# endernewton/tf-faster-rcnn

Measured on AMD Instinct MI355X. Metric: images/sec (600×1000) ResNet-101 Faster R-CNN at 1/2/4/8 MI355X, higher is better.
Workload: dtype f32 (operands, accumulators, results; GEMMs with Cin, Cout % 128 == 0 form each f32 product from two-piece fp16 operands with an exact power-of-two scale per 128-k block on the fp16 matrix pipe -- 3 MFMAs / product, dropped terms <= 3 * 2^-22, measured error vs float64 below the f32-MFMA kernel's; o

## Files before the change

### scratch/h2_conv3.py

```python
import os, sys
ROOT = os.path.dirname(os.path.dirname(os.path.abspath(__file__)))
sys.path[:0] = [os.path.join(ROOT, "tf-faster-rcnn_amd")]
args = [a for a in sys.argv[1:]]
lib_path, single = None, 0
if "--lib" in args:
    i = args.index("--lib"); lib_path = args[i + 1]; del args[i:i + 2]
if "--single" in args:
    i = args.index("--single"); single = int(args[i + 1]); del args[i:i + 2]
import frcnn_hip
if lib_path:
    frcnn_hip.LIB_PATH = os.path.abspath(lib_path)
import numpy as np, torch
from frcnn_hip import ops
dev = torch.device("cuda:0")
shapes = {
    "b4c3x8":  (1, 117600, 2048, 512, True, True, True, 0),
    "b4c3x8m": (8, 14700, 2048, 512, True, False, False, 49),
    "b4c3x8pm": (8, 14700, 2048, 512, "planes", False, False, 49),
    "b3c3x8":  (1, 19152, 1024, 256, True, True, True, 0),
    "b2c3x8":  (1, 75000, 512, 128, True, True, True, 0),
    "b4c3x8p": (1, 117600, 2048, 512, "planes", False, True, 0),
    "b3c3x8p": (1, 19152, 1024, 256, "planes", False, True, 0),
    "b3scx8":  (1, 19152, 1024, 512, False, True, True, 0),
    "w7x8":    (121, 2400, 512, 512, False, True, False, 0),
    "w3x8":    (36, 1280, 256, 256, False, True, False, 0),
    "wrpnx8":  (36, 1280, 512, 1024, False, True, False, 0),
    "b4c1x8":  (1, 117600, 512, 2048, False, False, True, 0),
    "b3c1x8":  (1, 19152, 256, 1024, False, True, False, 0),
    "cal_k128": (1, 117600, 128, 128, "planes", False, True, 0),
    "b4c3x1":  (1, 14700, 2048, 512, True, True, True, 0),
    "b3c3x1":  (1, 2394, 1024, 256, True, True, True, 0),
}
cfgs = [int(c) for c in (args[0] if args else "9,21,12").split(",")]
only = args[1].split(",") if len(args) > 1 else ["b4c3x8", "b4c3x8m", "b3c3x8", "b2c3x8", "w7x8", "w3x8", "b4c1x8", "b3c1x8"]
if not single:
    print("%-8s %-4s %9s %9s %8s %8s  %s" % ("shape", "cfg", "med_us", "min_us", "TFLOP/s", "GB/s", "bits vs cfg %d" % cfgs[0]))
for name in only:
    G, M, N, K, has_res, f32o, planes, mean_rows = shapes[name]
    torch.manual_seed(1)
    x = torch.randn(G * M, K, device=dev).clamp(min=0) * torch.exp(torch.rand(G * M, K, device=dev) * 4 - 2)
    shared_w = mean_rows > 0
    w = torch.randn(1 if shared_w else G, N, K, device=dev) * 0.05
    b = torch.randn(N, device=dev) if (G == 1 or shared_w) else None
    res = torch.randn(G * M, N, device=dev) if has_res else None
    if has_res == "planes":
        res = ops.h2_split(res.clamp(min=0))
    xp, wp = ops.h2_split(x), ops.h2_pack_w(w)
    del x
    outs, outp = {}, {}
    share = G * M * N * 4 > (1 << 29)
    for c in cfgs:
        if mean_rows:
            outs[c] = torch.empty(G * M // mean_rows, N, device=dev)
        else:
            outs[c] = (outs[cfgs[0]] if (share and c != cfgs[0]) else torch.empty(G * M, N, device=dev)) if f32o else None
            outp[c] = (outp[cfgs[0]] if (share and c != cfgs[0]) else ops.H2.empty(G * M, N, dev)) if planes else None

    def run(c):
        if mean_rows:
            return ops.gemm_h2_mean(xp, wp, G, M, N, K, b, res, 1, mean_rows, out=outs[c], cfg=c)
        return ops.gemm_h2(xp, wp, G, M, N, K, b, res, 1, out=outs[c], out_planes=outp.get(c), want_f32=f32o, cfg=c)

    if single:
        for _ in range(single):
            run(cfgs[0])
        torch.cuda.synchronize()
        break
    def digest(c):
        parts = []
        if outs.get(c) is not None:
            parts.append(outs[c].view(torch.int32).to(torch.int64).sum())
            parts.append((outs[c].view(torch.int32).to(torch.int64) * torch.arange(1, outs[c].numel() + 1, device=dev).view(outs[c].shape) % 1000003).sum())
        if outp.get(c) is not None:
            pv = outp[c].planes.view(torch.int16).to(torch.int64)
            parts.append(pv.sum()); parts.append((pv * (torch.arange(pv.numel(), device=dev) % 8191 + 1)).sum())
            parts.append(outp[c].inv.view(torch.int32).to(torch.int64).sum())
        return tuple(int(p) for p in parts)
    digs = {}
    for c in cfgs:
        if outs.get(c) is not None: outs[c].fill_(float("nan"))
        if outp.get(c) is not None: outp[c].planes.zero_(); outp[c].inv.zero_()
        try:
            run(c); torch.cuda.synchronize()
            digs[c] = digest(c)
        except Exception as e:
            digs[c] = "unsupported (%s)" % (str(e)[:60],)
    live = [c for c in cfgs if not isinstance(digs[c], str)]
    times = {c: [] for c in live}
    for r in range(6):
        for c in live:
            e0, e1 = torch.cuda.Event(enable_timing=True), torch.cuda.Event(enable_timing=True)
            e0.record()
            for _ in range(6): run(c)
            e1.record(); torch.cuda.synchronize()
            if r: times[c].append(e0.elapsed_time(e1) * 1000 / 6)
    nbytes = 4.0 * G * M * K + 4.0 * (w.numel()) + G * M * N * 4.0 * ((1 if has_res else 0) + (1 if f32o else 0) + (1 if planes else 0))
    for c in cfgs:
        if c not in live:
            print("%-8s %-4d %s" % (name, c, digs[c]), flush=True)
            continue
        med = float(np.median(times[c]))
        print("%-8s %-4d %9.1f %9.1f %8.1f %8.0f  %s" % (name, c, med, min(times[c]), 2.0 * G * M * N * K / med / 1e6, nbytes / med / 1e3,
                                                       "identical" if digs[c] == digs[cfgs[0]] else "DIFFERENT"), flush=True)
    del outs, outp, xp, res
    torch.cuda.empty_cache()
```

### tf-faster-rcnn_amd/csrc/gemm_h2.hip

```cpp
#include "h2_common.h"
#include <mutex>
#include <type_traits>

typedef float f32x16 __attribute__((ext_vector_type(16)));
typedef _Float16 h8 __attribute__((ext_vector_type(8)));

#define LDS_AS __attribute__((address_space(3)))

struct GemmH2Params {
  const unsigned short* x; const float* x_inv; const unsigned short* w; const float* w_inv;
  const float* bias; const float* res; const unsigned short* resp; const float* resp_inv; float* y; unsigned short* yp; float* y_inv;
  int M, N, K, batch, act, nsteps, mtiles, ntiles;
  long long Mtot;
  int wshare;
  const float* mask;
  float* mean_part; int mean_rows;
};

__device__ __forceinline__ void h2_glds16(unsigned voff, const void* sbase, unsigned lds_base) {
  unsigned keep;
  asm volatile(
      "s_mov_b32 %0, m0\n\t"
      "s_mov_b32 m0, %3\n\t"
      "s_nop 0\n\t"
// ... 318 lines not shown
  };

  int c_tile = tile0, c_step = 0, cur = 0, nxt = 0;
  int c_bm0 = 0, c_bn0 = 0, c_g = 0;
  auto set_ctile = [&](int tl) {
    int g, mt, nt;
    tile_coords(tl, g, mt, nt);
    c_bm0 = mt * BM; c_bn0 = nt * BN; c_g = g;
  };
  const float act_lo = p.act == FRCNN_ACT_NONE ? -__builtin_inff() : 0.f;
  const float act_hi = p.act == FRCNN_ACT_RELU6 ? 6.f : __builtin_inff();

  auto rsrc_f = [&](const void* base, long long elems_left, int esize) {
    const long long bytes = elems_left * esize;
    return __builtin_amdgcn_make_buffer_rsrc((void*)base, 0, (int)max(0ll, min(bytes, 0x7fffffffll)), 0x00020000);
  };

  struct TileRef { int bm0, bn0, g, cpar; };
  auto ent_rsrc = [&](const void* base, int g, int esize) {
    const char* b = (const char*)base + (size_t)g * p.M * p.N * esize;
    return __builtin_amdgcn_make_buffer_rsrc((void*)b, 0, p.M * p.N * esize, 0x00020000);
  };
  const int lo4 = (frow * p.N + 4 * khalf) * 4;
  auto lo2_of = [&]() { int v = lo4; asm volatile("" : "+v"(v)); return v >> 1; };
  auto lo2w_of = [&]() { int v = lo4; asm volatile("" : "+v"(v)); return (v >> 1) + 8 * (int)(threadIdx.x >> 5 & 1); };
  auto sub_off = [&](const auto& T, int i, int j) {
    return __builtin_amdgcn_readfirstlane((T.bm0 + wm0 + i * 32) * p.N + T.bn0 + wn0 + j * 32);
  };

  auto load_res_raw = [&](int i) {
    typedef unsigned u32x4 __attribute__((ext_vector_type(4)));
    const TileRef C{c_bm0, c_bn0, c_g, c_cpar};
    const bool planes = !p.res && p.resp;
    const auto none = __builtin_amdgcn_make_buffer_rsrc((void*)nullptr, 0, 0, 0x00020000);
    const auto r_even = p.res ? ent_rsrc(p.res, c_g, 4) : planes ? ent_rsrc(p.resp, c_g, 2) : none;
    const auto r_odd = p.res ? r_even : planes ? ent_rsrc(p.resp + (size_t)p.Mtot * p.N, c_g, 2) : none;
    const int step_q = planes ? 0 : 32, step_p = planes ? 32 : 0;
    int base = lo4;
    asm volatile("" : "+v"(base));
    if (planes) base = (base >> 1) + 8 * (int)(threadIdx.x >> 5 & 1);
#pragma unroll
    for (int j = 0; j < TN; ++j) {
      const int vo = base + sub_off(C, i, j) * (planes ? 2 : 4);
#pragma unroll
      for (int q = 0; q < 4; ++q) {
        const u32x4 ld = __builtin_amdgcn_raw_buffer_load_b128((q & 1) ? r_odd : r_even, vo, q * step_q + (q >> 1) * step_p, 0);
        tot[i][j][4 * q + 0] = __uint_as_float(ld[0]); tot[i][j][4 * q + 1] = __uint_as_float(ld[1]);
        tot[i][j][4 * q + 2] = __uint_as_float(ld[2]); tot[i][j][4 * q + 3] = __uint_as_float(ld[3]);
      }
      pend += 4;
    }
  };
  auto init_tot = [&]() {
    if constexpr (DE) return;
    if constexpr (LTB) {
      if (p.res || p.resp) {
#pragma unroll
        for (int i = 0; i < TM; ++i) load_res_raw(i);
      } else {
#pragma unroll
        for (int i = 0; i < TM; ++i)
#pragma unroll
          for (int j = 0; j < TN; ++j)
#pragma unroll
            for (int r = 0; r < 16; ++r) tot[i][j][r] = 0.f;
      }
      return;
    }
    const size_t row_base = (size_t)c_g * p.M;
    typedef unsigned u32x4 __attribute__((ext_vector_type(4)));
    if (p.res) {
#pragma unroll
      for (int i = 0; i < TM; ++i)
#pragma unroll
        for (int j = 0; j < TN; ++j) {
          const int m0 = c_bm0 + wm0 + i * 32, nc = c_bn0 + wn0 + j * 32;
          const auto rr = rsrc_f(p.res + (long long)(row_base + m0) * p.N + nc, (long long)(p.M - m0) * p.N - nc, 4);
#pragma unroll
          for (int q = 0; q < 4; ++q) {
            const u32x4 ld = __builtin_amdgcn_raw_buffer_load_b128(rr, (frow * p.N + 4 * khalf) * 4 + 32 * q, 0, 0);
            tot[i][j][4 * q + 0] = __uint_as_float(ld[0]); tot[i][j][4 * q + 1] = __uint_as_float(ld[1]);
            tot[i][j][4 * q + 2] = __uint_as_float(ld[2]); tot[i][j][4 * q + 3] = __uint_as_float(ld[3]);
          }
        }
      pend += TM * TN * 4;
    } else if (p.resp) {
      float ri[TM];
#pragma unroll
      for (int i = 0; i < TM; ++i)
        ri[i] = p.resp_inv[(size_t)(c_bn0 / H2_KB) * p.Mtot + row_base + min(c_bm0 + wm0 + i * 32 + frow, p.M - 1)];
      h4 hv[TM][TN][4], lv[TM][TN][4];
#pragma unroll
      for (int i = 0; i < TM; ++i)
#pragma unroll
        for (int j = 0; j < TN; ++j) {
          const int m0 = c_bm0 + wm0 + i * 32, nc = c_bn0 + wn0 + j * 32;
          const long long sbase = (long long)(row_base + m0) * p.N + nc, left_e = (long long)(p.M - m0) * p.N - nc;
          const auto rh = rsrc_f(p.resp + sbase, left_e, 2), rl = rsrc_f(p.resp + (size_t)p.Mtot * p.N + sbase, left_e, 2);
#pragma unroll
          for (int q = 0; q < 4; ++q) {
            const int lo2 = (frow * p.N + 4 * khalf) * 2 + 16 * q;
            hv[i][j][q] = __builtin_bit_cast(h4, __builtin_amdgcn_raw_buffer_load_b64(rh, lo2, 0, 0));
            lv[i][j][q] = __builtin_bit_cast(h4, __builtin_amdgcn_raw_buffer_load_b64(rl, lo2, 0, 0));
          }
        }
#pragma unroll
      for (int i = 0; i < TM; ++i)
#pragma unroll
        for (int j = 0; j < TN; ++j)
#pragma unroll
          for (int q = 0; q < 4; ++q)
#pragma unroll
            for (int e = 0; e < 4; ++e) tot[i][j][4 * q + e] = ((float)hv[i][j][q][e] + (float)lv[i][j][q][e]) * ri[i];
    } else {
#pragma unroll
      for (int i = 0; i < TM; ++i)
#pragma unroll
        for (int j = 0; j < TN; ++j)
#pragma unroll
          for (int r = 0; r < 16; ++r) tot[i][j][r] = 0.f;
    }
    float4 wi[TN][4], bv[TN][4];
#pragma unroll
    for (int j = 0; j < TN; ++j)
#pragma unroll
      for (int q = 0; q < 4; ++q)
        wi[j][q] = *(const float4*)(p.w_inv + (size_t)(p.wshare ? 0 : c_g) * p.N + c_bn0 + wn0 + j * 32 + 4 * khalf + 8 * q);
    if (p.bias) {
#pragma unroll
      for (int j = 0; j < TN; ++j)
#pragma unroll
        for (int q = 0; q < 4; ++q) bv[j][q] = *(const float4*)(p.bias + c_bn0 + wn0 + j * 32 + 4 * khalf + 8 * q);
    } else {
#pragma unroll
      for (int j = 0; j < TN; ++j)
#pragma unroll
        for (int q = 0; q < 4; ++q) bv[j][q] = make_float4(0.f, 0.f, 0.f, 0.f);
    }
#pragma unroll
    for (int j = 0; j < TN; ++j)
#pragma unroll
      for (int q = 0; q < 4; ++q) {
        const float s0 = __uint_as_float(0x7f000000u - __float_as_uint(wi[j][q].x)), s1 = __uint_as_float(0x7f000000u - __float_as_uint(wi[j][q].y));
        const float s2 = __uint_as_float(0x7f000000u - __float_as_uint(wi[j][q].z)), s3 = __uint_as_float(0x7f000000u - __float_as_uint(wi[j][q].w));
#pragma unroll
        for (int i = 0; i < TM; ++i) {
          tot[i][j][4 * q + 0] = (tot[i][j][4 * q + 0] + bv[j][q].x) * s0;
          tot[i][j][4 * q + 1] = (tot[i][j][4 * q + 1] + bv[j][q].y) * s1;
          tot[i][j][4 * q + 2] = (tot[i][j][4 * q + 2] + bv[j][q].z) * s2;
          tot[i][j][4 * q + 3] = (tot[i][j][4 * q + 3] + bv[j][q].w) * s3;
        }
      }
  };

  auto ep_scale_act = [&](const TileRef& T) {
#pragma unroll
    for (int j = 0; j < TN; ++j) {
      const int n0 = T.bn0 + wn0 + j * 32 + 4 * khalf;
#pragma unroll
      for (int q = 0; q < 4; ++q) {
        const float4 wi = LTB ? *(const float4*)(smem + CB_OFF + T.cpar * (2 * BN * 4) + (wn0 + j * 32 + 4 * khalf + 8 * q) * 4)
                             : *(const float4*)(p.w_inv + (size_t)(p.wshare ? 0 : T.g) * p.N + n0 + 8 * q);
#pragma unroll
        for (int i = 0; i < TM; ++i) {
          tot[i][j][4 * q + 0] = act_clamp(tot[i][j][4 * q + 0] * wi.x, act_lo, act_hi);
          tot[i][j][4 * q + 1] = act_clamp(tot[i][j][4 * q + 1] * wi.y, act_lo, act_hi);
          tot[i][j][4 * q + 2] = act_clamp(tot[i][j][4 * q + 2] * wi.z, act_lo, act_hi);
          tot[i][j][4 * q + 3] = act_clamp(tot[i][j][4 * q + 3] * wi.w, act_lo, act_hi);
        }
      }
    }
  };
  auto ep_mask = [&](const TileRef& T) {
    if (MASKED && p.mask) {
      const auto rk = ent_rsrc(p.mask, T.g, 4);
#pragma unroll
      for (int i = 0; i < TM; ++i)
#pragma unroll
        for (int j = 0; j < TN; ++j) {
          const int vo = lo4 + sub_off(T, i, j) * 4;
          typedef unsigned u32x4 __attribute__((ext_vector_type(4)));
          u32x4 k[4];
#pragma unroll
          for (int q = 0; q < 4; ++q) k[q] = __builtin_amdgcn_raw_buffer_load_b128(rk, vo + 32 * q, 0, 0);
#pragma unroll
          for (int q = 0; q < 4; ++q)
#pragma unroll
            for (int e = 0; e < 4; ++e) tot[i][j][4 * q + e] = __uint_as_float(k[q][e]) > 0.f ? tot[i][j][4 * q + e] : 0.f;
        }
      pend += TM * TN * 4;
    }
  };
  auto ep_mean = [&](const TileRef& T, int i) {
    const int mb = T.bm0 + wm0 + i * 32;
    if (mb >= p.M) return;
    const int nblk = (p.M + 31) >> 5;
    const int m = mb + frow, g0 = mb / p.mean_rows, gid = m / p.mean_rows;
    const bool in_a = m < p.M && gid == g0, in_b = m < p.M && gid == g0 + 1;
    const bool two = mb - g0 * p.mean_rows + 31 >= p.mean_rows;
    float* dst = p.mean_part + ((size_t)T.g * nblk + (mb >> 5)) * 2 * p.N;
#pragma unroll
    for (int j = 0; j < TN; ++j) {
      const int n0 = T.bn0 + wn0 + j * 32 + 4 * khalf;
#pragma unroll
      for (int q = 0; q < 4; ++q) {
        float a[4];
#pragma unroll
        for (int e = 0; e < 4; ++e) a[e] = h2_sum32(in_a ? tot[i][j][4 * q + e] : 0.f);
        if (frow == 0) *(float4*)(dst + n0 + 8 * q) = make_float4(a[0], a[1], a[2], a[3]);
        ++pend;
        if (two) {
          float b[4];
#pragma unroll
          for (int e = 0; e < 4; ++e) b[e] = h2_sum32(in_b ? tot[i][j][4 * q + e] : 0.f);
          if (frow == 0) *(float4*)(dst + p.N + n0 + 8 * q) = make_float4(b[0], b[1], b[2], b[3]);
          ++pend;
        }
      }
    }
  };
  auto ep_store_f32 = [&](const TileRef& T, int i) {
    if (!p.y) return;
    const auto ry = ent_rsrc(p.y, T.g, 4);
#pragma unroll
    for (int j = 0; j < TN; ++j) {
      const int lo = lo4 + sub_off(T, i, j) * 4;
#pragma unroll
      for (int q = 0; q < 4; ++q) {
        typedef unsigned u32x4 __attribute__((ext_vector_type(4)));
        u32x4 o;
        o[0] = __float_as_uint(tot[i][j][4 * q + 0]); o[1] = __float_as_uint(tot[i][j][4 * q + 1]);
        o[2] = __float_as_uint(tot[i][j][4 * q + 2]); o[3] = __float_as_uint(tot[i][j][4 * q + 3]);
        __builtin_amdgcn_raw_buffer_store_b128(o, ry, lo + 32 * q, 0, 0);
      }
      pend += 4;
      if constexpr (DE) __builtin_amdgcn_sched_barrier(0);
    }
  };
  auto ep_rowmax_write = [&](float (&mx)[TM]) {
    float* red = (float*)(smem + RED_OFF);
#pragma unroll
    for (int i = 0; i < TM; ++i) {
      float m = 0.f;
#pragma unroll
      for (int j = 0; j < TN; ++j)
#pragma unroll
        for (int r = 0; r < 16; ++r) m = fmaxf(m, fabsf(tot[i][j][r]));
      m = fmaxf(m, __shfl_xor(m, 32, 64));
      mx[i] = m;
      if (BN / WN > 1 && khalf == 0) red[wni * BM + wm0 + i * 32 + frow] = m;
    }
  };
  auto ep_rowmax_merge = [&](float (&mx)[TM]) {
    const float* red = (const float*)(smem + RED_OFF);
#pragma unroll
    for (int i = 0; i < TM; ++i)
#pragma unroll
      for (int o = 0; o < BN / WN; ++o) mx[i] = fmaxf(mx[i], red[o * BM + wm0 + i * 32 + frow]);
  };
  auto ep_store_planes = [&](const TileRef& T, int i, float mxi) {
    const size_t row_base = (size_t)T.g * p.M;
    const size_t yplane = (size_t)p.Mtot * p.N;
    float scale, inv;
    h2_block_scale(mxi, scale, inv);
    const int m0 = T.bm0 + wm0 + i * 32;
    if (wni == 0 && khalf == 0 && m0 + frow < p.M)
      p.y_inv[(size_t)(T.bn0 / H2_KB) * p.Mtot + row_base + m0 + frow] = inv;
    const auto rh = ent_rsrc(p.yp, T.g, 2), rl = ent_rsrc(p.yp + yplane, T.g, 2);
#pragma unroll
    for (int j = 0; j < TN; ++j) {
      const int so = sub_off(T, i, j) * 2;
      typedef unsigned u32x2 __attribute__((ext_vector_type(2)));
      if constexpr (W21) {
        const int lo = lo2w_of() + so;
#pragma unroll
        for (int pq = 0; pq < 2; ++pq) {
          h4 ha, la, hb, lb;
          h2_split4(make_float4(tot[i][j][8 * pq + 0], tot[i][j][8 * pq + 1], tot[i][j][8 * pq + 2], tot[i][j][8 * pq + 3]), scale, ha, la);
          h2_split4(make_float4(tot[i][j][8 * pq + 4], tot[i][j][8 * pq + 5], tot[i][j][8 * pq + 6], tot[i][j][8 * pq + 7]), scale, hb, lb);
          const u32x2 uha = __builtin_bit_cast(u32x2, ha), uhb = __builtin_bit_cast(u32x2, hb);
          const u32x2 ula = __builtin_bit_cast(u32x2, la), ulb = __builtin_bit_cast(u32x2, lb);
          typedef unsigned u32x4 __attribute__((ext_vector_type(4)));
          const auto h0 = __builtin_amdgcn_permlane32_swap(uha[0], uhb[0], false, false), h1 = __builtin_amdgcn_permlane32_swap(uha[1], uhb[1], false, false);
          const auto l0 = __builtin_amdgcn_permlane32_swap(ula[0], ulb[0], false, false), l1 = __builtin_amdgcn_permlane32_swap(ula[1], ulb[1], false, false);
          __builtin_amdgcn_raw_buffer_store_b128(u32x4{h0[0], h1[0], h0[1], h1[1]}, rh, lo + 32 * pq, 0, 0);
          __builtin_amdgcn_raw_buffer_store_b128(u32x4{l0[0], l1[0], l0[1], l1[1]}, rl, lo + 32 * pq, 0, 0);
        }
        pend += 4;
        if constexpr (DE) __builtin_amdgcn_sched_barrier(0);
      } else {
        const int lo = lo2_of() + so;
#pragma unroll
        for (int q = 0; q < 4; ++q) {
          h4 hh, ll;
          h2_split4(make_float4(tot[i][j][4 * q + 0], tot[i][j][4 * q + 1], tot[i][j][4 * q + 2], tot[i][j][4 * q + 3]), scale, hh, ll);
          __builtin_amdgcn_raw_buffer_store_b64(__builtin_bit_cast(u32x2, hh), rh, lo + 16 * q, 0, 0);
          __builtin_amdgcn_raw_buffer_store_b64(__builtin_bit_cast(u32x2, ll), rl, lo + 16 * q, 0, 0);
        }
        pend += 8;
      }
    }
  };

  auto epilogue = [&]() {
    const TileRef T{c_bm0, c_bn0, c_g, c_cpar};
    ep_scale_act(T);
    ep_mask(T);
    if (p.mean_part) {
#pragma unroll
      for (int i = 0; i < TM; ++i) ep_mean(T, i);
      c_cpar ^= 1;
      return;
    }
#pragma unroll
    for (int i = 0; i < TM; ++i) ep_store_f32(T, i);
    if (p.yp) {
      float mx[TM];
      ep_rowmax_write(mx);
      if (BN / WN > 1) {
        asm volatile("s_waitcnt lgkmcnt(0)" ::: "memory");
        __builtin_amdgcn_s_barrier();
        ep_rowmax_merge(mx);
      }
#pragma unroll
      for (int i = 0; i < TM; ++i) ep_store_planes(T, i, mx[i]);
      if (BN / WN > 1) {
        asm volatile("s_waitcnt lgkmcnt(0)" ::: "memory");
        __builtin_amdgcn_s_barrier();
      }
    }
    c_cpar ^= 1;
  };

  constexpr int HALF = (TM + 1) / 2;
  bool have_prev = false;
  TileRef P{0, 0, 0, 0};
  float dmx[TM];
  (void)dmx;
  auto de_piece = [&](auto pos_c) {
    constexpr int POS = decltype(pos_c)::value;
    if constexpr (POS == 0) {
      if (have_prev) {
        ep_scale_act(P);
        ep_mask(P);
        if (p.yp) ep_rowmax_write(dmx);
      }
    } else if constexpr (POS == 1 || POS == 2) {
      constexpr int I0 = POS == 1 ? 0 : HALF, I1 = POS == 1 ? HALF : TM;
      if (have_prev) {
        if (POS == 1 && p.yp && BN / WN > 1) ep_rowmax_merge(dmx);
#pragma unroll
        for (int i = I0; i < I1; ++i) {
          ep_store_f32(P, i);
          if (p.yp) ep_store_planes(P, i, dmx[i]);
        }
      }
#pragma unroll
      for (int i = I0; i < I1; ++i) load_res_raw(i);
    }
  };

  auto slab = [&](auto pos_c, bool fold, bool first_block) {
    constexpr int POS = decltype(pos_c)::value;
    const std::integral_constant<bool, POS == 0> first_c{};
    if constexpr (DE) asm volatile("s_waitcnt lgkmcnt(0)" ::: "memory");
    if constexpr (LTB) {
      wait_pending(pend);
    } else if (left >= 1) {
      if (wave == 0) h2_wait_vmcnt<(NS - 2) * (G + SL)>(); else h2_wait_vmcnt<(NS - 2) * G>();
    } else {
      h2_wait_vmcnt<0>();
    }
    __builtin_amdgcn_s_barrier();
    const bool more = left > 0;
    if (more) {
#pragma unroll
      for (int t = 0; t < (NO_LOAD ? 0 : G + SL); ++t) issue_one(nxt, t);
      if constexpr (LTB) {
        if (i_step == 0) issue_cb();
        pend = 0;
      }
    }
    if constexpr (DE) {
      __builtin_amdgcn_sched_barrier(0);
      if (first_block) de_piece(pos_c);
      __builtin_amdgcn_sched_barrier(0);
    }
    float ainv[TM];
    if (fold) {
      const int soff = ONCE ? S2_OFF + c_par * 1024 : cur * STAGE + S_OFF;
#pragma unroll
      for (int i = 0; i < TM; ++i) ainv[i] = *(const float*)(smem + soff + (wm0 + i * 32 + frow) * 4);
      c_par ^= 1;
    }
    slab_mfma(cur, first_c);
    if (more) {
      issue_advance();
      nxt = nxt + 1 == NS ? 0 : nxt + 1;
    }
    if (fold) {
      if (LTB && first_block) {
        const float* cbp = (const float*)(smem + CB_OFF + c_cpar * (2 * BN * 4));
        if (!p.res && p.resp) {
          typedef unsigned u32x2 __attribute__((ext_vector_type(2)));
#pragma unroll
          for (int i = 0; i < TM; ++i) {
            const float rri = *(const float*)(smem + c_cpar * STAGE + RI_OFF + (wm0 + i * 32 + frow) * 4);
#pragma unroll
            for (int j = 0; j < TN; ++j)
#pragma unroll
              for (int pq = 0; pq < 2; ++pq) {
                unsigned w[8];
#pragma unroll
                for (int e = 0; e < 8; ++e) w[e] = __float_as_uint(tot[i][j][8 * pq + e]);
                const auto h0 = __builtin_amdgcn_permlane32_swap(w[0], w[2], false, false), h1 = __builtin_amdgcn_permlane32_swap(w[1], w[3], false, false);
                const auto l0 = __builtin_amdgcn_permlane32_swap(w[4], w[6], false, false), l1 = __builtin_amdgcn_permlane32_swap(w[5], w[7], false, false);
                const h4 ha = __builtin_bit_cast(h4, u32x2{h0[0], h1[0]}), hb = __builtin_bit_cast(h4, u32x2{h0[1], h1[1]});
                const h4 la = __builtin_bit_cast(h4, u32x2{l0[0], l1[0]}), lb = __builtin_bit_cast(h4, u32x2{l0[1], l1[1]});
#pragma unroll
                for (int e = 0; e < 4; ++e) {
                  tot[i][j][8 * pq + e] = ((float)ha[e] + (float)la[e]) * rri;
                  tot[i][j][8 * pq + 4 + e] = ((float)hb[e] + (float)lb[e]) * rri;
                }
              }
          }
        }
#pragma unroll
        for (int j = 0; j < TN; ++j)
#pragma unroll
          for (int q = 0; q < 4; ++q) {
            const float4 wi = *(const float4*)(cbp + wn0 + j * 32 + 4 * khalf + 8 * q);
            const float4 bv = p.bias ? *(const float4*)(cbp + BN + wn0 + j * 32 + 4 * khalf + 8 * q) : make_float4(0.f, 0.f, 0.f, 0.f);
            const float s0 = __uint_as_float(0x7f000000u - __float_as_uint(wi.x)), s1 = __uint_as_float(0x7f000000u - __float_as_uint(wi.y));
            const float s2 = __uint_as_float(0x7f000000u - __float_as_uint(wi.z)), s3 = __uint_as_float(0x7f000000u - __float_as_uint(wi.w));
#pragma unroll
            for (int i = 0; i < TM; ++i) {
              tot[i][j][4 * q + 0] = __builtin_fmaf(tmp[i][j][4 * q + 0], ainv[i], (tot[i][j][4 * q + 0] + bv.x) * s0);
              tot[i][j][4 * q + 1] = __builtin_fmaf(tmp[i][j][4 * q + 1], ainv[i], (tot[i][j][4 * q + 1] + bv.y) * s1);
              tot[i][j][4 * q + 2] = __builtin_fmaf(tmp[i][j][4 * q + 2], ainv[i], (tot[i][j][4 * q + 2] + bv.z) * s2);
              tot[i][j][4 * q + 3] = __builtin_fmaf(tmp[i][j][4 * q + 3], ainv[i], (tot[i][j][4 * q + 3] + bv.w) * s3);
            }
          }
      } else {
#pragma unroll
        for (int i = 0; i < TM; ++i)
#pragma unroll
          for (int j = 0; j < TN; ++j)
#pragma unroll
            for (int r = 0; r < 16; ++r) tot[i][j][r] = __builtin_fmaf(tmp[i][j][r], ainv[i], tot[i][j][r]);
      }
    }
    cur = cur + 1 == NS ? 0 : cur + 1;
  };

  set_tile(i_tile);
  set_ctile(c_tile);
  if constexpr (PP) {
    const int grp = wave >> 2;
    h8 fxh[2][TM], fxl[2][TM], fwh[2][TN], fwl[2][TN];
    auto seg_barrier = [&]() {
      __builtin_amdgcn_sched_barrier(0);
      __builtin_amdgcn_s_barrier();
      __builtin_amdgcn_sched_barrier(0);
    };
    auto fold = [&]() {
      float ainv[TM];
#pragma unroll
      for (int i = 0; i < TM; ++i) ainv[i] = *(const float*)(smem + S2_OFF + (wave * 2 + c_par) * 256 + (i * 32 + frow) * 4);
      c_par ^= 1;
#pragma unroll
      for (int i = 0; i < TM; ++i)
#pragma unroll
        for (int j = 0; j < TN; ++j)
#pragma unroll
          for (int r = 0; r < 16; ++r) tot[i][j][r] = __builtin_fmaf(tmp[i][j][r], ainv[i], tot[i][j][r]);
    };
    auto pp_mem = [&](auto pos_c, bool fold_prev) -> bool {
      constexpr int POS = decltype(pos_c)::value;
      const char* sb = smem + cur * STAGE;
#pragma unroll
      for (int t = 0; t < 2; ++t) {
#pragma unroll
        for (int j = 0; j < TN; ++j) {
          const char* q = sb + w_row + j * 32 * 64 + (((2 * t + khalf) ^ sw) * 16);
          fwh[t][j] = __builtin_bit_cast(h8, *(const uint4*)(q));
          fwl[t][j] = __builtin_bit_cast(h8, *(const uint4*)(q + WP));
        }
#pragma unroll
        for (int i = 0; i < TM; ++i) {
          const char* q = sb + x_row + i * 32 * 64 + (((2 * t + khalf) ^ sw) * 16);
          fxh[t][i] = __builtin_bit_cast(h8, *(const uint4*)(q));
          fxl[t][i] = __builtin_bit_cast(h8, *(const uint4*)(q + XP));
        }
      }
      const bool more = left > 0;
      if (more) {
#pragma unroll
        for (int t = 0; t <= G; ++t) issue_one(nxt, t);
        issue_advance();
        nxt = nxt + 1 == NS ? 0 : nxt + 1;
      }
      if (fold_prev) fold();
      if (grp == 1) {
        if (more) h2_wait_vmcnt<(POS == 2 ? G + 1 : G)>(); else h2_wait_vmcnt<0>();
      }
      asm volatile("s_waitcnt lgkmcnt(0)" ::: "memory");
      seg_barrier();
      return more;
    };
    auto pp_mfma = [&](auto pos_c, bool issued) {
      constexpr int POS = decltype(pos_c)::value;
      __builtin_amdgcn_s_setprio(1);
#pragma unroll
      for (int t = 0; t < 2; ++t) {
#pragma unroll
        for (int i = 0; i < TM; ++i)
#pragma unroll
          for (int j = 0; j < TN; ++j) {
            if (POS == 0 && t == 0) {
              f32x16 z;
#pragma unroll
              for (int r = 0; r < 16; ++r) z[r] = 0.f;
              tmp[i][j] = __builtin_amdgcn_mfma_f32_32x32x16_f16(fwh[t][j], fxh[t][i], z, 0, 0, 0);
            } else {
              tmp[i][j] = __builtin_amdgcn_mfma_f32_32x32x16_f16(fwh[t][j], fxh[t][i], tmp[i][j], 0, 0, 0);
            }
          }
#pragma unroll
        for (int i = 0; i < TM; ++i)
#pragma unroll
          for (int j = 0; j < TN; ++j) tmp[i][j] = __builtin_amdgcn_mfma_f32_32x32x16_f16(fwl[t][j], fxh[t][i], tmp[i][j], 0, 0, 0);
#pragma unroll
        for (int i = 0; i < TM; ++i)
#pragma unroll
          for (int j = 0; j < TN; ++j) tmp[i][j] = __builtin_amdgcn_mfma_f32_32x32x16_f16(fwh[t][j], fxl[t][i], tmp[i][j], 0, 0, 0);
      }
      __builtin_amdgcn_s_setprio(0);
      if (grp == 0) {
        if (issued) h2_wait_vmcnt<(POS == 2 ? G + 1 : G)>(); else h2_wait_vmcnt<0>();
      }
      cur = cur + 1 == NS ? 0 : cur + 1;
      seg_barrier();
    };
    bool two = false;
#pragma unroll
    for (int s2 = 0; s2 < 2; ++s2) {
      if (left > 0) {
#pragma unroll
        for (int t = 0; t <= G; ++t) issue_one(nxt, t);
        issue_advance();
        nxt = nxt + 1 == NS ? 0 : nxt + 1;
        two = s2 == 1;
      }
    }
    if (two) h2_wait_vmcnt<G>(); else h2_wait_vmcnt<0>();
    seg_barrier();
    if (grp == 1) seg_barrier();
    const int nkb = p.nsteps >> 2;
    for (int tl = 0; tl < my_tiles; ++tl) {
      init_tot();
      for (int kb = 0; kb < nkb; ++kb) {
        bool is;
        is = pp_mem(std::integral_constant<int, 0>{}, kb > 0); pp_mfma(std::integral_constant<int, 0>{}, is);
        is = pp_mem(std::integral_constant<int, 1>{}, false);  pp_mfma(std::integral_constant<int, 1>{}, is);
        is = pp_mem(std::integral_constant<int, 2>{}, false);  pp_mfma(std::integral_constant<int, 2>{}, is);
        is = pp_mem(std::integral_constant<int, 3>{}, false);  pp_mfma(std::integral_constant<int, 3>{}, is);
      }
      fold();
      epilogue();
      c_tile += W8;
      if (tl + 1 < my_tiles) set_ctile(c_tile);
    }
    if (grp == 0) seg_barrier();
    h2_wait_vmcnt<0>();
    return;
  }
#pragma unroll
  for (int s = 0; s < NS - 1; ++s) {
    if (left > 0) {
#pragma unroll
      for (int t = 0; t < G + SL; ++t) issue_one(nxt, t);
      if constexpr (LTB) {
        if (i_step == 0) issue_cb();
        pend = 0;
      }
      issue_advance();
      nxt = nxt + 1 == NS ? 0 : nxt + 1;
    }
  }
  const int nkb = p.nsteps >> 2;
  for (int tl = 0; tl < my_tiles; ++tl) {
    init_tot();
    for (int kb = 0; kb < nkb; ++kb) {
      slab(std::integral_constant<int, 0>{}, false, kb == 0);
      slab(std::integral_constant<int, 1>{}, false, kb == 0);
      slab(std::integral_constant<int, 2>{}, false, kb == 0);
      slab(std::integral_constant<int, 3>{}, true, kb == 0);
    }
    if constexpr (DE) {
      if (tl + 1 < my_tiles) {
        P = TileRef{c_bm0, c_bn0, c_g, c_cpar};
        have_prev = true;
        c_cpar ^= 1;
        c_tile += W8;
        set_ctile(c_tile);
        continue;
      }
    }
    epilogue();
    c_tile += W8;
    if (tl + 1 < my_tiles) set_ctile(c_tile);
  }
  h2_wait_vmcnt<0>();
}

__global__ __launch_bounds__(256) void k_h2_split(const float* __restrict__ x, long long M, int K, unsigned short* __restrict__ planes,
                                                  float* __restrict__ inv_out) {
  const int nkb = K / H2_KB;
  const long long pairs = M * nkb;
  const int sub = threadIdx.x >> 5, l = threadIdx.x & 31;
  for (long long pr = (long long)blockIdx.x * 8 + sub; pr < pairs; pr += (long long)gridDim.x * 8) {
    const long long m = pr / nkb;
    const int kb = (int)(pr - m * nkb);
    const size_t e = (size_t)m * K + (size_t)kb * H2_KB + 4 * l;
    const float4 v = *(const float4*)(x + e);
    float mx = fmaxf(fmaxf(fabsf(v.x), fabsf(v.y)), fmaxf(fabsf(v.z), fabsf(v.w)));
#pragma unroll
    for (int o = 16; o >= 1; o >>= 1) mx = fmaxf(mx, __shfl_xor(mx, o, 64));
    float scale, inv;
    h2_block_scale(mx, scale, inv);
    h4 hh, ll;
    h2_split4(v, scale, hh, ll);
    *(h4*)(planes + e) = hh;
    *(h4*)(planes + (size_t)M * K + e) = ll;
    if (l == 0) inv_out[(size_t)kb * M + m] = inv;
  }
}

__global__ __launch_bounds__(256) void k_h2_pack_w(const float* __restrict__ w, int rows, int N, int K, unsigned short* __restrict__ planes,
                                                   float* __restrict__ inv_out) {
  const int row = blockIdx.x * 4 + (threadIdx.x >> 6), l = threadIdx.x & 63;
  if (row >= rows) return;
  const float* src = w + (size_t)row * K;
  float mx = 0.f;
  for (int k = 4 * l; k < K; k += 256) {
    const float4 v = *(const float4*)(src + k);
    mx = fmaxf(mx, fmaxf(fmaxf(fabsf(v.x), fabsf(v.y)), fmaxf(fabsf(v.z), fabsf(v.w))));
  }
#pragma unroll
  for (int o = 32; o >= 1; o >>= 1) mx = fmaxf(mx, __shfl_xor(mx, o, 64));
  float scale, inv;
  h2_block_scale(fmaxf(mx, 0x1p-40f), scale, inv);
  const int g = row / N, n = row - g * N;
  unsigned short* ph = planes + ((size_t)g * 2 * N + n) * K;
  unsigned short* pl = ph + (size_t)N * K;
  for (int k = 4 * l; k < K; k += 256) {
    const float4 v = *(const float4*)(src + k);
    h4 hh, ll;
    _Float16 a, b;
    h2_split1(v.x, scale, a, b); hh[0] = a; ll[0] = b;
    h2_split1(v.y, scale, a, b); hh[1] = a; ll[1] = b;
    h2_split1(v.z, scale, a, b); hh[2] = a; ll[2] = b;
    h2_split1(v.w, scale, a, b); hh[3] = a; ll[3] = b;
    *(h4*)(ph + k) = hh;
    *(h4*)(pl + k) = ll;
  }
  if (l == 0) inv_out[row] = inv;
}

extern "C" size_t frcnn_h2_planes_bytes(long long rows, int K) {
  if (rows <= 0 || K <= 0) return 0;
  return (size_t)2 * (size_t)rows * (size_t)K * sizeof(unsigned short);
}

extern "C" int frcnn_h2_pack_w(const float* w_d, int G, int N, int K, void* planes_d, float* w_inv_d, void* stream) {
  if (!w_d || !planes_d || !w_inv_d || G <= 0 || N <= 0 || K <= 0) return FRCNN_E_ARG;
  if (K % 4) return FRCNN_E_UNSUPPORTED;
  const int rows = G * N;
  hipLaunchKernelGGL(k_h2_pack_w, dim3((unsigned)cdiv(rows, 4)), dim3(256), 0, (hipStream_t)stream, w_d, rows, N, K, (unsigned short*)planes_d, w_inv_d);
  LAUNCH_CHECK();
  return FRCNN_OK;
}

extern "C" int frcnn_h2_split(const float* x_d, long long M, int K, void* planes_d, float* inv_d, void* stream) {
  if (!x_d || !planes_d || !inv_d || M <= 0 || K <= 0) return FRCNN_E_ARG;
  if (K % H2_KB) return FRCNN_E_UNSUPPORTED;
  const long long pairs = M * (K / H2_KB);
  const unsigned grid = (unsigned)min((pairs + 7) / 8, (long long)256 * 64);
  hipLaunchKernelGGL(k_h2_split, dim3(grid), dim3(256), 0, (hipStream_t)stream, x_d, M, K, (unsigned short*)planes_d, inv_d);
  LAUNCH_CHECK();
  return FRCNN_OK;
}

template <int BM, int BN, int WM, int WN, int NS, int WPE = 2, int TUNE = 0>
static int launch_h2(const GemmH2Params& q, hipStream_t st) {
  constexpr int NT = (BM / WM) * (BN / WN) * 64;
  constexpr size_t lds = H2Lds<BM, BN, WM, WN, NS, TUNE>::TOTAL;
  auto kern = k_gemm_h2<BM, BN, WM, WN, NS, WPE, TUNE>;
  static KernelOnce once;
  int slots = 0;
  HIP_TRY(kernel_once(once, (const void*)kern, NT, lds, &slots));
  if (slots < 8 || q.N % BN) return FRCNN_E_UNSUPPORTED;
  if (q.yp && BN != H2_KB) return FRCNN_E_UNSUPPORTED;
  GemmH2Params p = q;
  p.mtiles = cdiv(p.M, BM); p.ntiles = p.N / BN; p.nsteps = p.K / 32;
  const long long T = (long long)p.mtiles * p.ntiles * p.batch;
  if (T >= (1ll << 30)) return FRCNN_E_UNSUPPORTED;
  const int grid = (int)min((long long)(slots / 8) * 8, ((T + 7) / 8) * 8);
  hipLaunchKernelGGL(kern, dim3(grid), dim3(NT), lds, st, p);
  LAUNCH_CHECK();
  return FRCNN_OK;
}

template <int MASK>
static int h2_dispatch(const GemmH2Params& p, int cfg, hipStream_t st) {
  switch (cfg) {
    case 9: return launch_h2<128, 128, 64, 64, 2, 2, H2_SCALES_ONCE + MASK>(p, st);
    case 12: return launch_h2<64, 128, 32, 64, 2, 2, MASK>(p, st);
    case 21: return launch_h2<256, 128, 64, 64, 3, 2, H2_SCALES_ONCE + H2_PINGPONG + MASK>(p, st);
    case 30: return launch_h2<128, 128, 64, 64, 2, 2, H2_SCALES_ONCE + H2_LIGHT_BOUNDARY + MASK>(p, st);
    case 31: return launch_h2<128, 128, 64, 64, 2, 2, H2_SCALES_ONCE + H2_LIGHT_BOUNDARY + H2_STORE16 + MASK>(p, st);
    case 32: return launch_h2<128, 128, 64, 64, 2, 2, H2_SCALES_ONCE + H2_STORE16 + MASK>(p, st);
    case 33: return launch_h2<64, 128, 32, 64, 2, 2, H2_LIGHT_BOUNDARY + H2_STORE16 + MASK>(p, st);
    case 34: return launch_h2<256, 128, 64, 64, 3, 2, H2_SCALES_ONCE + H2_PINGPONG + H2_STORE16 + MASK>(p, st);
    case 40: return launch_h2<128, 128, 64, 64, 2, 2, H2_SCALES_ONCE + H2_LIGHT_BOUNDARY + H2_STORE16 + H2_DEFERRED + MASK>(p, st);
    case 41: return launch_h2<64, 128, 32, 64, 2, 2, H2_LIGHT_BOUNDARY + H2_STORE16 + H2_DEFERRED + MASK>(p, st);
  }
#ifdef FRCNN_ABLATION
  constexpr int CFG31 = H2_SCALES_ONCE + H2_LIGHT_BOUNDARY + H2_STORE16;
  if constexpr (MASK == 0) switch (cfg) {
    case 50: return launch_h2<128, 128, 64, 64, 2, 2, CFG31 + H2_NO_MFMA>(p, st);
    case 51: return launch_h2<128, 128, 64, 64, 2, 2, CFG31 + H2_NO_FRAG>(p, st);
    case 52: return launch_h2<128, 128, 64, 64, 2, 2, CFG31 + H2_NO_LOAD>(p, st);
    case 53: return launch_h2<128, 128, 64, 64, 2, 2, CFG31 + H2_NO_MFMA + H2_NO_FRAG>(p, st);
    case 54: return launch_h2<128, 128, 64, 64, 2, 2, CFG31 + H2_NO_FRAG + H2_NO_LOAD>(p, st);
    case 55: return launch_h2<128, 128, 64, 64, 2, 2, CFG31 + H2_NO_MFMA + H2_NO_FRAG + H2_NO_LOAD>(p, st);
  }
#endif
  return FRCNN_E_ARG;
}

static int run_h2(GemmH2Params& p, int cfg, hipStream_t st);

static GemmH2Params h2_params(const void* x_planes_d, const float* x_inv_d, const void* w_planes_d, const float* w_inv_d, const float* bias_d,
                              const float* res_d, const void* res_planes_d, const float* res_inv_d, float* y_d, void* y_planes_d, float* y_inv_d,
                              int G, int M, int N, int K, int act) {
  GemmH2Params p;
  p.x = (const unsigned short*)x_planes_d; p.x_inv = x_inv_d; p.w = (const unsigned short*)w_planes_d; p.w_inv = w_inv_d;
  p.bias = bias_d; p.res = res_d; p.resp = (const unsigned short*)res_planes_d; p.resp_inv = res_inv_d; p.y = y_d; p.yp = (unsigned short*)y_planes_d; p.y_inv = y_inv_d;
  p.M = M; p.N = N; p.K = K; p.batch = G; p.act = act; p.Mtot = (long long)G * M;
  p.nsteps = p.mtiles = p.ntiles = 0;
  p.mean_part = nullptr; p.mean_rows = 0; p.wshare = 0; p.mask = nullptr;
  return p;
}

extern "C" int frcnn_gemm_h2(const void* x_planes_d, const float* x_inv_d, const void* w_planes_d, const float* w_inv_d, const float* bias_d,
                             const float* res_d, const void* res_planes_d, const float* res_inv_d, float* y_d, void* y_planes_d, float* y_inv_d,
                             int G, int M, int N, int K, int act, int cfg, void* stream) {
  if (!x_planes_d || !x_inv_d || !w_planes_d || !w_inv_d || (!y_d && !y_planes_d) || (y_planes_d && !y_inv_d) || G <= 0 || M <= 0 || N <= 0 ||
      K <= 0 || act < 0 || act > 2 || (res_d && res_planes_d) || (res_planes_d && !res_inv_d))
    return FRCNN_E_ARG;
  const long long Mtot = (long long)G * M;
  if (K % H2_KB || N % 128 || 4ll * Mtot * K >= (1ll << 32) || 4ll * N * K >= (1ll << 32) ||
      (long long)M * N >= (1ll << 29))
    return FRCNN_E_UNSUPPORTED;
  GemmH2Params p = h2_params(x_planes_d, x_inv_d, w_planes_d, w_inv_d, bias_d, res_d, res_planes_d, res_inv_d, y_d, y_planes_d, y_inv_d, G, M, N, K, act);
  return run_h2(p, cfg, (hipStream_t)stream);
}

extern "C" int frcnn_gemm_h2_masked(const void* x_planes_d, const float* x_inv_d, const void* w_planes_d, const float* w_inv_d, const float* bias_d,
                                    const float* res_d, const float* mask_d, float* y_d, void* y_planes_d, float* y_inv_d, int G, int M, int N, int K,
                                    int act, int cfg, void* stream) {
  if (!x_planes_d || !x_inv_d || !w_planes_d || !w_inv_d || !mask_d || (!y_d && !y_planes_d) || (y_planes_d && !y_inv_d) || G <= 0 || M <= 0 ||
      N <= 0 || K <= 0 || act < 0 || act > 2)
    return FRCNN_E_ARG;
  const long long Mtot = (long long)G * M;
  if (K % H2_KB || N % 128 || 4ll * Mtot * K >= (1ll << 32) || 4ll * N * K >= (1ll << 32) || (long long)M * N >= (1ll << 29)) return FRCNN_E_UNSUPPORTED;
  GemmH2Params p = h2_params(x_planes_d, x_inv_d, w_planes_d, w_inv_d, bias_d, res_d, nullptr, nullptr, y_d, y_planes_d, y_inv_d, G, M, N, K, act);
  p.mask = mask_d;
  return run_h2(p, cfg, (hipStream_t)stream);
}

static int run_h2(GemmH2Params& p, int cfg, hipStream_t st) {
  const int G = p.batch, M = p.M, N = p.N, K = p.K;
  if (cfg < 0) {
    const long long mt256 = (M + 255) / 256;
#ifndef FRCNN_H2_PP_MIN_K
#define FRCNN_H2_PP_MIN_K 1024
#endif
    const int pp_min_k = ((cfg == -4 || cfg == -5 || cfg == -6) && !p.mean_part) ? 512 : FRCNN_H2_PP_MIN_K;
    const int pp_cfg = (cfg == -3 || cfg == -4 || (cfg == -6 && K < FRCNN_H2_PP_MIN_K)) ? 34 : 21;
    const bool pp = K >= pp_min_k && mt256 * 256 * 100 <= (long long)M * 104 && mt256 * (N / 128) * G >= 256;
    const bool tiny = (long long)((M + 127) / 128) * (N / 128) * G < 150;
    const bool de = cfg != -2 && cfg != -7 && !p.mean_part && !p.mask && ((p.resp && p.yp && !p.y) || cfg == -8);
    cfg = pp ? pp_cfg : tiny ? (cfg == -2 ? 12 : (de && cfg == -8) ? 41 : 33) : (cfg == -2 ? 9 : de ? 40 : 31);
  }
  if (p.mean_part && (cfg == 40 || cfg == 41)) cfg = cfg == 40 ? 31 : 33;
  return p.mask ? h2_dispatch<H2_MASKED>(p, cfg, st) : h2_dispatch<0>(p, cfg, st);
}

__global__ __launch_bounds__(256) void k_h2_mean_finish(const float* __restrict__ part, int G, int M, int N4, int rows, float4* __restrict__ out) {
  const long long t = (long long)blockIdx.x * blockDim.x + threadIdx.x;
  const int per = M / rows;
  if (t >= (long long)G * per * N4) return;
  const int n4 = (int)(t % N4);
  const long long gr = t / N4;
  const int g = (int)(gr / per), r = (int)(gr % per);
  const int nblk = (M + 31) >> 5;
  const int row0 = r * rows, row1 = row0 + rows - 1;
  float4 s = make_float4(0.f, 0.f, 0.f, 0.f);
  for (int b = row0 >> 5; b <= (row1 >> 5); ++b) {
    const int which = ((b << 5) / rows == r) ? 0 : 1;
    const float4 v = *(const float4*)(part + (((size_t)g * nblk + b) * 2 + which) * (size_t)N4 * 4 + (size_t)n4 * 4);
    s.x += v.x; s.y += v.y; s.z += v.z; s.w += v.w;
  }
  const float inv = 1.0f / (float)rows;
  out[t] = make_float4(s.x * inv, s.y * inv, s.z * inv, s.w * inv);
}

extern "C" size_t frcnn_gemm_h2_mean_workspace_bytes(int G, int M, int N) {
  if (G <= 0 || M <= 0 || N <= 0) return 256;
  return (size_t)G * (size_t)((M + 31) / 32) * 2 * (size_t)N * sizeof(float);
}

extern "C" int frcnn_gemm_h2_mean(const void* x_planes_d, const float* x_inv_d, const void* w_planes_d, const float* w_inv_d, const float* bias_d,
                                  const float* res_d, const void* res_planes_d, const float* res_inv_d, int G, int M, int N, int K, int act, int rows,
                                  float* mean_out_d, void* ws, size_t ws_bytes, int cfg, void* stream) {
  if (!x_planes_d || !x_inv_d || !w_planes_d || !w_inv_d || !mean_out_d || !ws || G <= 0 || M <= 0 || N <= 0 || K <= 0 || act < 0 || act > 2 ||
      rows <= 0 || (res_d && res_planes_d) || (res_planes_d && !res_inv_d))
    return FRCNN_E_ARG;
  const long long Mtot = (long long)G * M;
  if (K % H2_KB || N % 128 || M % rows || rows < 32 || 4ll * Mtot * K >= (1ll << 32) || 4ll * N * K >= (1ll << 32) || (long long)M * N >= (1ll << 29))
    return FRCNN_E_UNSUPPORTED;
  if (frcnn_gemm_h2_mean_workspace_bytes(G, M, N) > ws_bytes) return FRCNN_E_WS;
  GemmH2Params p = h2_params(x_planes_d, x_inv_d, w_planes_d, w_inv_d, bias_d, res_d, res_planes_d, res_inv_d, nullptr, nullptr, nullptr, G, M, N, K, act);
  p.mean_part = (float*)ws; p.mean_rows = rows; p.wshare = 1;
  hipStream_t st = (hipStream_t)stream;
  const int rc = run_h2(p, cfg, st);
  if (rc) return rc;
  const long long tot = (long long)G * (M / rows) * (N / 4);
  hipLaunchKernelGGL(k_h2_mean_finish, dim3((unsigned)((tot + 255) / 256)), dim3(256), 0, st, (const float*)ws, G, M, N / 4, rows, (float4*)mean_out_d);
  LAUNCH_CHECK();
  return FRCNN_OK;
}
```

Before: 550.3.

## Skip dead M-tiles in ping-pong GEMM and widen its auto-dispatch classes

```diff
diff --git a/scratch/h2_conv3.py b/scratch/h2_conv3.py
--- a/scratch/h2_conv3.py
+++ b/scratch/h2_conv3.py
@@ -19,6 +19,7 @@
     "b4c3x8pm": (8, 14700, 2048, 512, "planes", False, False, 49),
     "b3c3x8":  (1, 19152, 1024, 256, True, True, True, 0),
     "b2c3x8":  (1, 75000, 512, 128, True, True, True, 0),
+    "b4c3x8r": (1, 117600, 2048, 512, True, False, True, 0),
     "b4c3x8p": (1, 117600, 2048, 512, "planes", False, True, 0),
     "b3c3x8p": (1, 19152, 1024, 256, "planes", False, True, 0),
     "b3scx8":  (1, 19152, 1024, 512, False, True, True, 0),
diff --git a/tf-faster-rcnn_amd/csrc/gemm_h2.hip b/tf-faster-rcnn_amd/csrc/gemm_h2.hip
--- a/tf-faster-rcnn_amd/csrc/gemm_h2.hip
+++ b/tf-faster-rcnn_amd/csrc/gemm_h2.hip
@@ -644,28 +644,36 @@
     }
   };
 
-  auto epilogue = [&]() {
+  auto epilogue = [&](bool live) {
     const TileRef T{c_bm0, c_bn0, c_g, c_cpar};
-    ep_scale_act(T);
-    ep_mask(T);
+    if (live) {
+      ep_scale_act(T);
+      ep_mask(T);
+    }
     if (p.mean_part) {
-#pragma unroll
-      for (int i = 0; i < TM; ++i) ep_mean(T, i);
+      if (live) {
+#pragma unroll
+        for (int i = 0; i < TM; ++i) ep_mean(T, i);
+      }
       c_cpar ^= 1;
       return;
     }
-#pragma unroll
-    for (int i = 0; i < TM; ++i) ep_store_f32(T, i);
+    if (live) {
+#pragma unroll
+      for (int i = 0; i < TM; ++i) ep_store_f32(T, i);
+    }
     if (p.yp) {
       float mx[TM];
-      ep_rowmax_write(mx);
+      if (live) ep_rowmax_write(mx);
       if (BN / WN > 1) {
         asm volatile("s_waitcnt lgkmcnt(0)" ::: "memory");
         __builtin_amdgcn_s_barrier();
-        ep_rowmax_merge(mx);
-      }
-#pragma unroll
-      for (int i = 0; i < TM; ++i) ep_store_planes(T, i, mx[i]);
+        if (live) ep_rowmax_merge(mx);
+      }
+      if (live) {
+#pragma unroll
+        for (int i = 0; i < TM; ++i) ep_store_planes(T, i, mx[i]);
+      }
       if (BN / WN > 1) {
         asm volatile("s_waitcnt lgkmcnt(0)" ::: "memory");
         __builtin_amdgcn_s_barrier();
@@ -817,22 +825,32 @@
 #pragma unroll
           for (int r = 0; r < 16; ++r) tot[i][j][r] = __builtin_fmaf(tmp[i][j][r], ainv[i], tot[i][j][r]);
     };
-    auto pp_mem = [&](auto pos_c, bool fold_prev) -> bool {
+    auto pp_mem = [&](auto pos_c, bool fold_prev, bool live) -> bool {
       constexpr int POS = decltype(pos_c)::value;
       const char* sb = smem + cur * STAGE;
-#pragma unroll
-      for (int t = 0; t < 2; ++t) {
-#pragma unroll
-        for (int j = 0; j < TN; ++j) {
-          const char* q = sb + w_row + j * 32 * 64 + (((2 * t + khalf) ^ sw) * 16);
-          fwh[t][j] = __builtin_bit_cast(h8, *(const uint4*)(q));
-          fwl[t][j] = __builtin_bit_cast(h8, *(const uint4*)(q + WP));
-        }
-#pragma unroll
-        for (int i = 0; i < TM; ++i) {
-          const char* q = sb + x_row + i * 32 * 64 + (((2 * t + khalf) ^ sw) * 16);
-          fxh[t][i] = __builtin_bit_cast(h8, *(const uint4*)(q));
-          fxl[t][i] = __builtin_bit_cast(h8, *(const uint4*)(q + XP));
+      if (live) {
+#pragma unroll
+        for (int t = 0; t < 2; ++t) {
+#pragma unroll
+          for (int j = 0; j < TN; ++j) {
+            const char* q = sb + w_row + j * 32 * 64 + (((2 * t + khalf) ^ sw) * 16);
+            fwh[t][j] = __builtin_bit_cast(h8, *(const uint4*)(q));
+            fwl[t][j] = __builtin_bit_cast(h8, *(const uint4*)(q + WP));
+          }
+#pragma unroll
+          for (int i = 0; i < TM; ++i) {
+            const char* q = sb + x_row + i * 32 * 64 + (((2 * t + khalf) ^ sw) * 16);
+            fxh[t][i] = __builtin_bit_cast(h8, *(const uint4*)(q));
+            fxl[t][i] = __builtin_bit_cast(h8, *(const uint4*)(q + XP));
+          }
+        }
+      } else {
+#pragma unroll
+        for (int t = 0; t < 2; ++t) {
+#pragma unroll
+          for (int j = 0; j < TN; ++j) asm volatile("" : "=v"(fwh[t][j]), "=v"(fwl[t][j]));
+#pragma unroll
+          for (int i = 0; i < TM; ++i) asm volatile("" : "=v"(fxh[t][i]), "=v"(fxl[t][i]));
         }
       }
       const bool more = left > 0;
@@ -850,32 +868,34 @@
       seg_barrier();
       return more;
     };
-    auto pp_mfma = [&](auto pos_c, bool issued) {
+    auto pp_mfma = [&](auto pos_c, bool issued, bool live) {
       constexpr int POS = decltype(pos_c)::value;
       __builtin_amdgcn_s_setprio(1);
-#pragma unroll
-      for (int t = 0; t < 2; ++t) {
-#pragma unroll
-        for (int i = 0; i < TM; ++i)
-#pragma unroll
-          for (int j = 0; j < TN; ++j) {
-            if (POS == 0 && t == 0) {
-              f32x16 z;
-#pragma unroll
-              for (int r = 0; r < 16; ++r) z[r] = 0.f;
-              tmp[i][j] = __builtin_amdgcn_mfma_f32_32x32x16_f16(fwh[t][j], fxh[t][i], z, 0, 0, 0);
-            } else {
-              tmp[i][j] = __builtin_amdgcn_mfma_f32_32x32x16_f16(fwh[t][j], fxh[t][i], tmp[i][j], 0, 0, 0);
+      if (live) {
+#pragma unroll
+        for (int t = 0; t < 2; ++t) {
+#pragma unroll
+          for (int i = 0; i < TM; ++i)
+#pragma unroll
+            for (int j = 0; j < TN; ++j) {
+              if (POS == 0 && t == 0) {
+                f32x16 z;
+#pragma unroll
+                for (int r = 0; r < 16; ++r) z[r] = 0.f;
+                tmp[i][j] = __builtin_amdgcn_mfma_f32_32x32x16_f16(fwh[t][j], fxh[t][i], z, 0, 0, 0);
+              } else {
+                tmp[i][j] = __builtin_amdgcn_mfma_f32_32x32x16_f16(fwh[t][j], fxh[t][i], tmp[i][j], 0, 0, 0);
+              }
             }
-          }
-#pragma unroll
-        for (int i = 0; i < TM; ++i)
-#pragma unroll
-          for (int j = 0; j < TN; ++j) tmp[i][j] = __builtin_amdgcn_mfma_f32_32x32x16_f16(fwl[t][j], fxh[t][i], tmp[i][j], 0, 0, 0);
-#pragma unroll
-        for (int i = 0; i < TM; ++i)
-#pragma unroll
-          for (int j = 0; j < TN; ++j) tmp[i][j] = __builtin_amdgcn_mfma_f32_32x32x16_f16(fwh[t][j], fxl[t][i], tmp[i][j], 0, 0, 0);
+#pragma unroll
+          for (int i = 0; i < TM; ++i)
+#pragma unroll
+            for (int j = 0; j < TN; ++j) tmp[i][j] = __builtin_amdgcn_mfma_f32_32x32x16_f16(fwl[t][j], fxh[t][i], tmp[i][j], 0, 0, 0);
+#pragma unroll
+          for (int i = 0; i < TM; ++i)
+#pragma unroll
+            for (int j = 0; j < TN; ++j) tmp[i][j] = __builtin_amdgcn_mfma_f32_32x32x16_f16(fwh[t][j], fxl[t][i], tmp[i][j], 0, 0, 0);
+        }
       }
       __builtin_amdgcn_s_setprio(0);
       if (grp == 0) {
@@ -900,16 +920,23 @@
     if (grp == 1) seg_barrier();
     const int nkb = p.nsteps >> 2;
     for (int tl = 0; tl < my_tiles; ++tl) {
-      init_tot();
+      const bool live = __builtin_amdgcn_readfirstlane(c_bm0 + wm0 < p.M ? 1 : 0) != 0;
+      if (live) init_tot();
+      else {
+#pragma unroll
+        for (int i = 0; i < TM; ++i)
+#pragma unroll
+          for (int j = 0; j < TN; ++j) asm volatile("" : "=v"(tot[i][j]));
+      }
       for (int kb = 0; kb < nkb; ++kb) {
         bool is;
-        is = pp_mem(std::integral_constant<int, 0>{}, kb > 0); pp_mfma(std::integral_constant<int, 0>{}, is);
-        is = pp_mem(std::integral_constant<int, 1>{}, false);  pp_mfma(std::integral_constant<int, 1>{}, is);
-        is = pp_mem(std::integral_constant<int, 2>{}, false);  pp_mfma(std::integral_constant<int, 2>{}, is);
-        is = pp_mem(std::integral_constant<int, 3>{}, false);  pp_mfma(std::integral_constant<int, 3>{}, is);
-      }
-      fold();
-      epilogue();
+        is = pp_mem(std::integral_constant<int, 0>{}, live && kb > 0, live); pp_mfma(std::integral_constant<int, 0>{}, is, live);
+        is = pp_mem(std::integral_constant<int, 1>{}, false, live);          pp_mfma(std::integral_constant<int, 1>{}, is, live);
+        is = pp_mem(std::integral_constant<int, 2>{}, false, live);          pp_mfma(std::integral_constant<int, 2>{}, is, live);
+        is = pp_mem(std::integral_constant<int, 3>{}, false, live);          pp_mfma(std::integral_constant<int, 3>{}, is, live);
+      }
+      if (live) fold(); else c_par ^= nkb & 1;
+      epilogue(live);
       c_tile += W8;
       if (tl + 1 < my_tiles) set_ctile(c_tile);
     }
@@ -949,7 +976,7 @@
         continue;
       }
     }
-    epilogue();
+    epilogue(true);
     c_tile += W8;
     if (tl + 1 < my_tiles) set_ctile(c_tile);
   }
@@ -1083,6 +1110,9 @@
 }
 
 static int run_h2(GemmH2Params& p, int cfg, hipStream_t st);
+#ifndef FRCNN_H2_PP_CLASSES
+#define FRCNN_H2_PP_CLASSES 7
+#endif
 
 static GemmH2Params h2_params(const void* x_planes_d, const float* x_inv_d, const void* w_planes_d, const float* w_inv_d, const float* bias_d,
                               const float* res_d, const void* res_planes_d, const float* res_inv_d, float* y_d, void* y_planes_d, float* y_inv_d,
@@ -1126,15 +1156,28 @@
 static int run_h2(GemmH2Params& p, int cfg, hipStream_t st) {
   const int G = p.batch, M = p.M, N = p.N, K = p.K;
   if (cfg < 0) {
-    const long long mt256 = (M + 255) / 256;
+    const bool classes = cfg == -1;
+    if (cfg == -9) cfg = -1;
+    const long long mt256 = (M + 255) / 256, t256 = mt256 * (N / 128) * G;
 #ifndef FRCNN_H2_PP_MIN_K
 #define FRCNN_H2_PP_MIN_K 1024
 #endif
     const int pp_min_k = ((cfg == -4 || cfg == -5 || cfg == -6) && !p.mean_part) ? 512 : FRCNN_H2_PP_MIN_K;
-    const int pp_cfg = (cfg == -3 || cfg == -4 || (cfg == -6 && K < FRCNN_H2_PP_MIN_K)) ? 34 : 21;
-    const bool pp = K >= pp_min_k && mt256 * 256 * 100 <= (long long)M * 104 && mt256 * (N / 128) * G >= 256;
+    int pp_cfg = (cfg == -3 || cfg == -4 || (cfg == -6 && K < FRCNN_H2_PP_MIN_K)) ? 34 : 21;
+    const bool waste256_ok = mt256 * 256 * 100 <= (long long)M * 104;
+    bool pp = K >= pp_min_k && waste256_ok && t256 >= 256;
+    bool to31 = false;
+    if (classes && !p.mean_part && !p.mask) {
+      const long long m64 = (M + 63) / 64 * 64;
+      const bool waste64_ok = m64 * 100 <= (long long)M * 104;
+      const bool products = (FRCNN_H2_PP_CLASSES & 1) && G > 1 && p.y && !p.yp && !p.res && !p.resp && K >= 512 && waste64_ok && t256 >= 256;
+      const bool conv3_f32res = (FRCNN_H2_PP_CLASSES & 2) && p.res && p.yp && K == 512 && waste64_ok && t256 >= 256;
+      if (conv3_f32res && !pp) pp_cfg = 34;
+      pp = pp || products || conv3_f32res;
+      to31 = (FRCNN_H2_PP_CLASSES & 4) && p.resp && p.yp && !p.y && K == 512;
+    }
     const bool tiny = (long long)((M + 127) / 128) * (N / 128) * G < 150;
-    const bool de = cfg != -2 && cfg != -7 && !p.mean_part && !p.mask && ((p.resp && p.yp && !p.y) || cfg == -8);
+    const bool de = cfg != -2 && cfg != -7 && !p.mean_part && !p.mask && ((p.resp && p.yp && !p.y) || cfg == -8) && !to31;
     cfg = pp ? pp_cfg : tiny ? (cfg == -2 ? 12 : (de && cfg == -8) ? 41 : 33) : (cfg == -2 ? 9 : de ? 40 : 31);
   }
   if (p.mean_part && (cfg == 40 || cfg == 41)) cfg = cfg == 40 ? 31 : 33;
```

Result: faster. 558.6, median of 6 (+1.5%).
